# breuner/elbencho

Hardware: AMD Instinct MI355X
Metric: seq-read GiB/s into GPU HBM (higher is better)
Workload: dtype raw-bytes; 1 GPU; seqread; model=storage-benchmark seq-read into HBM, threads_per_gpu=16, block_size=4194304, iodepth=1, bench_dir=/dev/shm/elbencho_amd_bench, gpu_staged=True, mmap_zero_copy=True, dynamic_slice=True, verify_on_gpu=True, verify_salt=7, parallelism=single, device=AMD Radeon Graphics, device_numa_node=0

## Files before the change

elbencho_amd/csrc/engine.cpp:

```cpp

#include "engine.h"

#include <fcntl.h>
#include <linux/fs.h>
#include <pthread.h>
#include <sched.h>
#include <sys/ioctl.h>
#include <sys/mman.h>
#include <sys/stat.h>
#include <sys/types.h>
#include <unistd.h>

#include <algorithm>
#include <random>
#include <cerrno>
#include <cstdio>
#include <cstring>

#include "netbench.h"
#include "uring.h"

namespace eb {

static constexpr uint64_t INTERRUPT_CHECK_INTERVAL = 128;
// ... 884 lines not shown
                if (slotBusy[slot]) gpu->waitSlotEvent(slot);
                if (lat && gpu->timedPairActive(slot))
                    addIoLat(preadUs[slot] + gpu->timedElapsedUSec(slot));

                auto t0 = lat ? Clock::now() : Clock::time_point();
                ssize_t res = pread(fg.fds[fileIdx], hostBufs[slot], ioLen, inFileOff);
                if (res != (ssize_t)ioLen) throwErrno("read", cfg.paths[fileIdx]);
                if (lat) {
                    preadUs[slot] = (uint64_t)std::chrono::duration_cast<
                        std::chrono::microseconds>(Clock::now() - t0).count();
                    gpu->recordTimedStart(slot);
                }

                gpu->copyH2DAsync(slot, ioLen);
                if (lat) gpu->recordTimedEnd(slot);
                if (doVerify) {
                    if ((inFileOff % 8 == 0) && (ioLen % 16 == 0)) {
                        if (eng.verifyMix)
                            gpu->verifyChecksumMixDevAsync(slot, ioLen, inFileOff,
                                                           (uint64_t)cfg.verifySalt,
                                                           cfg.blockSize, eng.verifyMixLen);
                        else
                            gpu->verifyChecksumDevAsync(slot, ioLen, inFileOff,
                                                        (uint64_t)cfg.verifySalt);
                        if (++sinceFetch >= VERIFY_FETCH_INTERVAL) {
                            fetchVerify();
                            sinceFetch = 0;
                        }
                    } else {
                        uint64_t bad =
                            eng.verifyMix
                                ? verifyChecksumMixCPU(hostBufs[slot], ioLen, inFileOff,
                                                       (uint64_t)cfg.verifySalt,
                                                       cfg.blockSize, eng.verifyMixLen)
                                : verifyChecksumCPU(hostBufs[slot], ioLen, inFileOff,
                                                    (uint64_t)cfg.verifySalt);
                        if (bad != UINT64_MAX)
                            throw WorkerError(
                                "Data verification failed. First bad file offset: " +
                                std::to_string(bad));
                    }
                }
                gpu->recordSlotEvent(slot);
                slotBusy[slot] = 1;

                liveOps.bytes.fetch_add(ioLen, std::memory_order_relaxed);
                liveOps.iops.fetch_add(1, std::memory_order_relaxed);
                slot = (slot + 1) % nSlots;
            }
            if (doVerify) fetchVerify();
            if (lat) {
                gpu->syncStream();
                for (int s = 0; s < nSlots; s++)
                    if (gpu->timedPairActive(s))
                        addIoLat(preadUs[s] + gpu->timedElapsedUSec(s));
            }
        }

        gpu->syncStream();
        return;
    }

    const bool lat = cfg.measureLat;
    BlockSpec spec;
    uint64_t opCount = 0;

    while (gen->next(spec)) {
        if ((opCount++ % INTERRUPT_CHECK_INTERVAL) == 0) checkInterrupt();

        uint64_t fileIdx, inFileOff, ioLen;
        if (!mapBlock(spec, fileIdx, inFileOff, ioLen)) continue;

        bool mixRead = rwMixActive &&
                       (isDedicatedReader ||
                        (cfg.rwMixThreads == 0 && rwMixDecideRead()));
        bool blockWrite = isWrite && !mixRead;

        if (rwMixActive && rwBalancerActive()) rwBalanceWait(mixRead, ioLen);

        auto t0 = lat ? Clock::now() : Clock::time_point();

        ssize_t res = blockIO(blockWrite, fg.fds[fileIdx], 0, ioLen, inFileOff,
                              mg.base(fileIdx), &cfg.paths[fileIdx]);
        if (res < 0)
            throwErrno(blockWrite ? "write" : "read", cfg.paths[fileIdx]);
        if ((uint64_t)res != ioLen)
            throw WorkerError(std::string("unexpected short ") + (blockWrite ? "write" : "read") +
                              ". Path: " + cfg.paths[fileIdx] +
                              "; expected: " + std::to_string(ioLen) +
                              "; got: " + std::to_string(res) +
                              (mixRead ? "; Hint: rwmix reads need a pre-written file." : ""));

        if (lat)
            addIoLat((uint64_t)std::chrono::duration_cast<std::chrono::microseconds>(
                Clock::now() - t0).count(), mixRead);

        AtomicLiveOps& ops = mixRead ? liveOpsReadMix : liveOps;
        ops.bytes.fetch_add(ioLen, std::memory_order_relaxed);
        ops.iops.fetch_add(1, std::memory_order_relaxed);
        if (rwMixActive && rwBalancerActive()) rwBalanceAccount(mixRead, ioLen);
    }

    if (isWrite && cfg.fsyncPerFile)
        for (size_t i = 0; i < fg.fds.size(); i++)
            if (fsync(fg.fds[i])) throwErrno("fsync", cfg.paths[i]);
}

void Worker::fileModeBlocksGpuMmap(bool isWrite)
{
    const auto& cfg = eng.cfg;
    const uint64_t fileSize = eng.effFileSize;
    const uint64_t bs = cfg.blockSize;
    const size_t numFiles = cfg.paths.size();
    const uint64_t numBlocksPerFile = (fileSize + bs - 1) / bs;
    const bool doVerify = cfg.verifySalt >= 0;
    const bool lat = cfg.measureLat;

    std::vector<char*> bases(numFiles);
    for (size_t i = 0; i < numFiles; i++)
        bases[i] = eng.getMappedReg(cfg.paths[i], fileSize, isWrite).base;

    const uint64_t mapBPF = (cfg.random || cfg.strided) ? (fileSize / bs) : numBlocksPerFile;
    const uint64_t virtFileLen = mapBPF * bs;

    const bool dynamic = cfg.dynamicSlice && !cfg.random && !cfg.strided &&
                         !cfg.backward && cfg.numThreads == cfg.numDataSetThreads;

    std::unique_ptr<OffsetGen> gen;
    if (dynamic) {
    } else if (cfg.random || cfg.strided) {
        uint64_t numBlocksTotal = mapBPF * numFiles;
        uint64_t rangeLen = bs * (numBlocksTotal / cfg.numDataSetThreads);
        uint64_t rangeOff = (uint64_t)globalRank * rangeLen;
        if (cfg.strided) {
            gen = std::make_unique<OffsetGenStrided>(bs, globalRank, cfg.numDataSetThreads);
            gen->reset(0, bs * numBlocksTotal);
        } else {
            gen = makeOffsetGen(rangeOff, rangeLen);
        }
    } else {
        uint64_t myStart, myLen;
        fairShareSlice(virtFileLen * numFiles, myStart, myLen);
        if (!myLen) return;
        gen = makeOffsetGen(myStart, myLen);
    }

    const int nSlots = (int)hostBufs.size();
    constexpr uint64_t VERIFY_FETCH_INTERVAL = 64;
    uint64_t sinceFetch = 0;
    BlockSpec spec;
    uint64_t opCount = 0;
    int slot = 0;

    auto fetchVerify = [&]() {
        GpuVerifyResult r = gpu->fetchVerifyResult();
        if (r.numMismatches)
            throw WorkerError("Data verification failed (GPU). First bad file offset: " +
                              std::to_string(r.firstBadFileOffset) +
                              "; mismatching 8-byte words: " +
                              std::to_string(r.numMismatches));
    };

    if (doVerify && !isWrite) (void)gpu->fetchVerifyResult();

    const uint64_t totalBlocks = numBlocksPerFile * numFiles;

    auto nextBlock = [&](uint64_t& fileIdx, uint64_t& inFileOff,
                         uint64_t& ioLen) -> bool {
        if (dynamic) {
            for (;;) {
                uint64_t b = eng.dynCursor.fetch_add(1, std::memory_order_relaxed);
                if (b >= totalBlocks) return false;
                fileIdx = b / numBlocksPerFile;
                inFileOff = (b % numBlocksPerFile) * bs;
                if (inFileOff >= fileSize) continue;
                ioLen = std::min(bs, fileSize - inFileOff);
                return true;
            }
        }
        while (gen->next(spec)) {
            if (!virtFileLen) return false;
            fileIdx = spec.offset / virtFileLen;
            if (fileIdx >= numFiles) continue;
            inFileOff = spec.offset - fileIdx * virtFileLen;
            if (inFileOff >= fileSize) continue;
            ioLen = std::min(spec.len, fileSize - inFileOff);
            return true;
        }
        return false;
    };

    uint64_t fileIdx, inFileOff, ioLen;
    while (nextBlock(fileIdx, inFileOff, ioLen)) {
        if ((opCount++ % INTERRUPT_CHECK_INTERVAL) == 0) checkInterrupt();

        rateLimiter.wait(ioLen);

        if (lat && gpu->timedPairActive(slot))
            addIoLat(gpu->timedElapsedUSec(slot));

        if (isWrite) {
            preWriteFill(slot, ioLen, inFileOff);
            if (lat) gpu->recordTimedStart(slot);
            gpu->copyToHostAsync(slot, bases[fileIdx] + inFileOff, ioLen);
            if (lat) gpu->recordTimedEnd(slot);
        } else {
            if (lat) gpu->recordTimedStart(slot);
            gpu->copyFromHostAsync(slot, bases[fileIdx] + inFileOff, ioLen);
            if (lat) gpu->recordTimedEnd(slot);
            if (doVerify && (inFileOff % 8 == 0) && (ioLen % 16 == 0)) {
                if (eng.verifyMix)
                    gpu->verifyChecksumMixDevAsync(slot, ioLen, inFileOff,
                                                   (uint64_t)cfg.verifySalt, cfg.blockSize,
                                                   eng.verifyMixLen);
                else
                    gpu->verifyChecksumDevAsync(slot, ioLen, inFileOff,
                                                (uint64_t)cfg.verifySalt);
                if (++sinceFetch >= VERIFY_FETCH_INTERVAL) {
                    fetchVerify();
                    sinceFetch = 0;
                }
            } else if (doVerify) {
                uint64_t bad =
                    eng.verifyMix
                        ? verifyChecksumMixCPU(bases[fileIdx] + inFileOff, ioLen, inFileOff,
                                               (uint64_t)cfg.verifySalt, cfg.blockSize,
                                               eng.verifyMixLen)
                        : verifyChecksumCPU(bases[fileIdx] + inFileOff, ioLen, inFileOff,
                                            (uint64_t)cfg.verifySalt);
                if (bad != UINT64_MAX)
                    throw WorkerError("Data verification failed. First bad file offset: " +
                                      std::to_string(bad));
            }
        }

        liveOps.bytes.fetch_add(ioLen, std::memory_order_relaxed);
        liveOps.iops.fetch_add(1, std::memory_order_relaxed);
        slot = (slot + 1) % nSlots;

        if ((opCount & 127) == 0) gpu->syncStream();
    }

    gpu->syncStream();
    if (lat)
        for (int s = 0; s < nSlots; s++)
            if (gpu->timedPairActive(s)) addIoLat(gpu->timedElapsedUSec(s));
    if (doVerify && !isWrite) fetchVerify();
}

void Worker::fileModeBlocksUring(bool isWrite)
{
    const auto& cfg = eng.cfg;
    const uint64_t fileSize = eng.effFileSize;
    const uint64_t bs = cfg.blockSize;
    const size_t numFiles = cfg.paths.size();
    const uint64_t numBlocksPerFile = (fileSize + bs - 1) / bs;
    const int depth = cfg.ioDepth;
    const bool lat = cfg.measureLat;

    const bool rwMixActive = isWrite && (cfg.rwMixPct > 0 || isDedicatedReader);

    FdGuard fg;
    int rwFlags = isWrite ? ((cfg.verifyDirect || rwMixActive) ? O_RDWR : O_WRONLY) : O_RDONLY;
    int openFlags = rwFlags | (cfg.directIO ? O_DIRECT : 0);
    if (isWrite && cfg.pathType == PathType::FILE) openFlags |= O_CREAT;
    for (const auto& p : cfg.paths) {
        int fd = open(p.c_str(), openFlags, 0644);
        if (fd < 0) throwErrno("open", p);
        fg.fds.push_back(fd);
        if (isWrite && cfg.pathType == PathType::FILE) {
            if (cfg.truncate && ftruncate(fd, 0)) throwErrno("truncate", p);
            if (cfg.truncToSize != UINT64_MAX && ftruncate(fd, fileSize))
                throwErrno("truncate-to-size", p);
            if (cfg.preallocFile && fallocate(fd, 0, 0, fileSize)) throwErrno("fallocate", p);
        }
        applyFadvise(fd, cfg.fadviseFlags, p);
    }

    const uint64_t mapBPF = (cfg.random || cfg.strided) ? (fileSize / bs) : numBlocksPerFile;
    const uint64_t virtFileLen = mapBPF * bs;

    auto mapBlock = [&](const BlockSpec& s, uint64_t& fileIdx, uint64_t& inFileOff,
                        uint64_t& ioLen) -> bool {
        if (!virtFileLen) return false;
        fileIdx = s.offset / virtFileLen;
        if (fileIdx >= numFiles) return false;
        inFileOff = s.offset - fileIdx * virtFileLen;
        if (inFileOff >= fileSize) return false;
        ioLen = std::min(s.len, fileSize - inFileOff);
        return true;
    };

    std::unique_ptr<OffsetGen> gen;
    if (cfg.random || cfg.strided) {
        uint64_t numBlocksTotal = mapBPF * numFiles;
        uint64_t rangeLen = bs * (numBlocksTotal / cfg.numDataSetThreads);
        uint64_t rangeOff = (uint64_t)globalRank * rangeLen;
        if (cfg.strided) {
            gen = std::make_unique<OffsetGenStrided>(bs, globalRank, cfg.numDataSetThreads);
            gen->reset(0, bs * numBlocksTotal);
        } else {
            gen = makeOffsetGen(rangeOff, rangeLen);
        }
    } else {
        uint64_t myStart, myLen;
        fairShareSlice(virtFileLen * numFiles, myStart, myLen);
        if (!myLen) return;
        gen = makeOffsetGen(myStart, myLen);
    }

    IoUring ring;
    ring.init(depth);

    if (!getenv("EB_URING_NOFIXED")) {
        std::vector<struct iovec> iovs(depth);
        for (int s = 0; s < depth; s++)
            iovs[s] = {hostBufs[s], (size_t)bs};
        ring.registerBuffers(iovs.data(), depth);
        ring.registerFiles(fg.fds.data(), (unsigned)fg.fds.size());
    }

    const int gpuBatch = gpu ? gpuBatchSlots(bs) : 1;
    const bool batchedRead = gpu && !isWrite && cfg.verifySalt < 0 &&
                             gpuBatch >= 2 && depth >= 4 &&
                             getenv("EB_GPU_URING_BATCH");
    if (getenv("EB_DEBUG_PATH"))
        fprintf(stderr, "[eb] uring path: gpu=%d batchedRead=%d batch=%d depth=%d\n",
                gpu ? 1 : 0, (int)batchedRead, gpuBatch, depth);
    if (batchedRead) {
        const int halfSize = std::min(depth / 2, 64);
        struct Op {
            uint64_t off = 0, len = 0;
            Clock::time_point start;
            int fileIdx = 0;
        };
        std::vector<Op> ops(2 * halfSize);
        std::vector<IoUring::Completion> bcomps(depth);
        int submitted[2] = {0, 0}, done[2] = {0, 0};
        bool exhausted2 = false;
        BlockSpec bspec;

        auto fillHalf = [&](int h) -> int {
            int base = h * halfSize;
            int n = 0;
            while (n < halfSize && !exhausted2) {
                uint64_t fileIdx = 0, inFileOff = 0, ioLen = 0;
                for (;;) {
                    if (!gen->next(bspec)) { exhausted2 = true; break; }
                    if (mapBlock(bspec, fileIdx, inFileOff, ioLen)) break;
                }
                if (exhausted2) break;
                rateLimiter.wait(ioLen);
                int slot = base + n;
                ops[slot] = {inFileOff, ioLen,
                             lat ? Clock::now() : Clock::time_point(), (int)fileIdx};
                if (eng.opsLog.isEnabled())
                    eng.opsLog.log(globalRank, "uring_read", cfg.paths[fileIdx],
                                   inFileOff, ioLen, true, false);
                int rfd = ring.hasFixedFiles() ? (int)fileIdx : fg.fds[fileIdx];
                while (!ring.prep(false, rfd, hostBufs[slot], ioLen, inFileOff,
                                  (uint64_t)slot,
                                  ring.hasFixedBuffers() ? slot : -1,
                                  ring.hasFixedFiles())) {
                    ring.submitAndWait(0);
                    checkInterrupt();
                }
                n++;
            }
            submitted[h] = n;
            done[h] = 0;
            return n;
        };

        int inFlightB = fillHalf(0) + fillHalf(1);
        uint64_t opCountB = 0;
        while (inFlightB > 0) {
            checkInterrupt();
            ring.submitAndWait(1, 250);
            unsigned n = ring.reap(bcomps.data(), depth);
            for (unsigned i = 0; i < n; i++) {
                int slot = (int)bcomps[i].userData;
                const Op& op = ops[slot];
                if (eng.opsLog.isEnabled())
                    eng.opsLog.log(globalRank, "uring_read", cfg.paths[op.fileIdx],
                                   op.off, op.len, false, bcomps[i].res < 0);
                if (bcomps[i].res < 0)
                    throw WorkerError(std::string("async read failed. Path: ") +
                                      cfg.paths[op.fileIdx] + "; SysErr: " +
                                      strerror(-bcomps[i].res));
                if ((uint64_t)bcomps[i].res != op.len)
                    throw WorkerError("unexpected short async read. Path: " +
                                      cfg.paths[op.fileIdx]);
                if (lat)
                    addIoLat((uint64_t)std::chrono::duration_cast<
                        std::chrono::microseconds>(Clock::now() - op.start).count());
                liveOps.bytes.fetch_add(op.len, std::memory_order_relaxed);
                liveOps.iops.fetch_add(1, std::memory_order_relaxed);
                done[slot / halfSize]++;
                inFlightB--;
                if ((opCountB++ % INTERRUPT_CHECK_INTERVAL) == 0) checkInterrupt();
// ... 1752 lines not shown
```

elbencho_amd/csrc/gpu.h:

```cpp

#pragma once

#include <cstdint>
#include <string>
#include <vector>

#include "crc.h"

namespace eb {

struct GpuVerifyResult {
    uint64_t numMismatches;
    uint64_t firstBadFileOffset;
};

void gpuHostRegister(void* ptr, uint64_t len);
bool gpuHostRegisterTry(void* ptr, uint64_t len);
void gpuHostUnregister(void* ptr);

class GpuCtx;

int gpuDeviceCount();

double gpuVerifyBenchGBs(uint64_t len, int iters, bool lds, int dev);

double gpuMixBenchGBs(uint64_t len, int iters, int dev, uint64_t blockSize, uint64_t mixLen,
                      bool fill, bool plainFill);

uint64_t gpuCrcTileBytes();
uint64_t gpuCrcWaveBytes();

std::string gpuProbeError();

std::string gpuDeviceName(int deviceId);

int gpuNumaNode(int deviceId);

class GpuCtx {
public:
    GpuCtx(int deviceId, int numSlots, uint64_t bufSize, bool pinnedHostBufs);
    ~GpuCtx();
    GpuCtx(const GpuCtx&) = delete;
    GpuCtx& operator=(const GpuCtx&) = delete;

    int deviceId() const { return devId; }
    char* hostBuf(int slot) const;
    uint64_t bufSize() const { return slotSize; }
    int numSlots() const { return slots; }
    uint64_t slotStride() const;

    void snapshotSlots(std::vector<char>& dst);

    void bindThread();

    void copyFromHostAsync(int slot, const void* src, uint64_t len);
    void copyToHostAsync(int slot, void* dst, uint64_t len);
    void copyH2DAsync(int slot, uint64_t len);
    void copyH2DRangeAsync(int firstSlot, int count);
    void copyD2HAsync(int slot, uint64_t len);
    void syncStream();

    void recordSlotEvent(int slot);
    void waitSlotEvent(int slot);

    void recordTimedStart(int slot);
    void recordTimedEnd(int slot);
    bool timedPairActive(int slot) const;
    uint64_t timedElapsedUSec(int slot);
    void dropTimedPairs();

    void verifyChecksumDevAsync(int slot, uint64_t len, uint64_t fileOff, uint64_t salt,
                                bool ldsVariant = false);
    GpuVerifyResult fetchVerifyResult();


    void fillRandDev(int slot, uint64_t len, uint64_t seed, bool fastAlgo = false);

    void fillChecksumDev(int slot, uint64_t len, uint64_t fileOff, uint64_t salt);

    GpuVerifyResult verifyChecksumDev(int slot, uint64_t len, uint64_t fileOff, uint64_t salt,
                                      bool ldsVariant = false);

    void fillChecksumMixDev(int slot, uint64_t len, uint64_t fileOff, uint64_t salt,
                            uint64_t blockSize, uint64_t mixLen);
    void verifyChecksumMixDevAsync(int slot, uint64_t len, uint64_t fileOff, uint64_t salt,
                                   uint64_t blockSize, uint64_t mixLen);
    GpuVerifyResult verifyChecksumMixDev(int slot, uint64_t len, uint64_t fileOff,
                                         uint64_t salt, uint64_t blockSize, uint64_t mixLen);

    void blockVarRefillDev(int slot, uint64_t len, uint64_t refillLen, uint64_t seed,
                           bool fastAlgo = false);


    void crcDevAsync(int slot, uint64_t len, CrcAlgo algo, uint64_t partialBase);

    uint32_t crcFetch(CrcAlgo algo, uint64_t totalLen, uint64_t tileCount);

    uint32_t crcDev(int slot, uint64_t len, CrcAlgo algo);

private:
    struct Impl;
    Impl* impl;
    int devId;
    uint64_t slotSize;
    int slots;
};

}
```

elbencho_amd/csrc/gpu_kernels.hip:

```cpp

#include <hip/hip_runtime.h>

#include <cstdio>
#include <map>
#include <mutex>
#include <stdexcept>
#include <string>
#include <vector>

#include "crc.h"
#include "gpu.h"

namespace eb {

#define HIP_CHECK(cmd)                                                                 \
    do {                                                                               \
        hipError_t e = (cmd);                                                          \
        if (e != hipSuccess)                                                           \
            throw std::runtime_error(std::string("HIP error: ") + hipGetErrorString(e) \
                                     + " at " __FILE__ ":" + std::to_string(__LINE__)); \
    } while (0)


__device__ __forceinline__ uint64_t d_splitmix64(uint64_t& state)
// ... 388 lines not shown
        ((uint4*)tab)[i] = ((const uint4*)tables)[i];
    __syncthreads();

    constexpr uint64_t TILE_VEC2 = CRC_TILE_BYTES / 16;
    const uint64_t nTiles = (nVec2 + TILE_VEC2 - 1) / TILE_VEC2;
    const int wave = threadIdx.x >> 6;
    const int lane = threadIdx.x & 63;

    for (uint64_t tile = blockIdx.x; tile < nTiles; tile += gridDim.x) {
        const uint64_t first = tile * TILE_VEC2;
        const uint64_t have = (nVec2 - first < TILE_VEC2) ? nVec2 - first : TILE_VEC2;
        const uint64_t pad = TILE_VEC2 - have;

        ulonglong2 v[CRC_STEPS_PER_WAVE];
#pragma unroll
        for (int j = 0; j < CRC_STEPS_PER_WAVE; j++) {
            uint64_t pos = (uint64_t)(wave * CRC_STEPS_PER_WAVE + j) * 64 + lane;
            v[j] = make_ulonglong2(0, 0);
            if (pos >= pad) v[j] = buf[first + pos - pad];
        }

        uint32_t acc = 0;
#pragma unroll
        for (int j = 0; j < CRC_STEPS_PER_WAVE; j++) {
            uint32_t r = 0;
#pragma unroll
            for (int k = 0; k < 8; k++) {
                r ^= tab[(CRC_TAB_ELEM + k) * 256 + ((v[j].x >> (8 * k)) & 0xFF)];
                r ^= tab[(CRC_TAB_ELEM + 8 + k) * 256 + ((v[j].y >> (8 * k)) & 0xFF)];
            }
            acc = d_crcLut4(tab + CRC_TAB_ROW * 256, acc) ^ r;
        }

#pragma unroll
        for (int i = 0; i < 6; i++) {
            uint32_t other = __shfl_down(acc, 1 << i, 64);
            acc = d_crcLut4(tab + (CRC_TAB_LANE + 4 * i) * 256, acc) ^ other;
        }

        if (lane == 0) wavePart[wave] = acc;
        __syncthreads();
        if (threadIdx.x == 0) {
            uint32_t t = 0;
#pragma unroll
            for (int w = 0; w < CRC_WAVES_PER_TILE; w++)
                t = d_crcLut4(tab + CRC_TAB_WAVE * 256, t) ^ wavePart[w];
            partial[tile] = t;
        }
        __syncthreads();
    }
}


double gpuVerifyBenchGBs(uint64_t len, int iters, bool lds, int dev);

bool gpuHostRegisterTry(void* ptr, uint64_t len)
{
    return hipHostRegister(ptr, len, hipHostRegisterDefault) == hipSuccess;
}

void gpuHostRegister(void* ptr, uint64_t len)
{
    HIP_CHECK(hipHostRegister(ptr, len, hipHostRegisterDefault));
}

void gpuHostUnregister(void* ptr) { (void)hipHostUnregister(ptr); }

int gpuDeviceCount()
{
    int n = 0;
    hipError_t e = hipGetDeviceCount(&n);
    if (e != hipSuccess) return 0;
    return n;
}

std::string gpuProbeError()
{
    int n = 0;
    hipError_t e = hipGetDeviceCount(&n);
    if (e != hipSuccess) return hipGetErrorString(e);
    return "ok: " + std::to_string(n) + " device(s)";
}

std::string gpuDeviceName(int deviceId)
{
    hipDeviceProp_t prop;
    if (hipGetDeviceProperties(&prop, deviceId) != hipSuccess) return "";
    return prop.name;
}

int gpuNumaNode(int deviceId)
{
    char busId[32] = {0};
    if (hipDeviceGetPCIBusId(busId, sizeof(busId), deviceId) != hipSuccess)
        return -1;
    for (char* c = busId; *c; ++c) *c = (char)tolower(*c);
    std::string path = std::string("/sys/bus/pci/devices/") + busId + "/numa_node";
    FILE* f = fopen(path.c_str(), "r");
    if (!f) return -1;
    int node = -1;
    if (fscanf(f, "%d", &node) != 1) node = -1;
    fclose(f);
    return node;
}

static dim3 gridForBytes(uint64_t workItems)
{
    uint64_t blocks = (workItems + 255) / 256;
    if (blocks > 4096) blocks = 4096;
    if (blocks == 0) blocks = 1;
    return dim3((uint32_t)blocks);
}

static hipStream_t sharedStream(int devId, int& poolSizeOut)
{
    static std::mutex mtx;
    static std::map<int, std::vector<hipStream_t>> pools;
    static std::map<int, int> next;
    static const int poolSize = [] {
        const char* v = getenv("EB_GPU_SHARED_STREAMS");
        int n = v ? atoi(v) : 8;
        return (n >= 1 && n <= 64) ? n : 0;
    }();

    poolSizeOut = poolSize;
    if (!poolSize) return nullptr;

    std::lock_guard<std::mutex> lk(mtx);
    auto& pool = pools[devId];
    if (pool.empty()) {
        pool.resize(poolSize);
        for (int i = 0; i < poolSize; i++)
            HIP_CHECK(hipStreamCreateWithFlags(&pool[i], hipStreamNonBlocking));
    }
    return pool[next[devId]++ % poolSize];
}

struct GpuCtx::Impl {
    hipStream_t stream = nullptr;
    bool ownStream = true;
    char* devBase = nullptr;
    char* hostBase = nullptr;
    uint64_t slotStride = 0;
    std::vector<char*> devBufs;
    std::vector<char*> hostBufs;
    std::vector<hipEvent_t> slotEvents;
    std::vector<hipEvent_t> timedStart, timedEnd;
    std::vector<char> timedActive;
    bool hostPinned = false;
    unsigned long long* verifyOutDev = nullptr;
    unsigned long long* verifyOutHost = nullptr;
    uint64_t fillCallCounter = 0;
    bool verifyDirty = false;

    uint32_t* crcTabDev[2] = {nullptr, nullptr};
    CrcShift crcTileShift[2];
    uint32_t* crcPartDev = nullptr;
    uint32_t* crcPartHost = nullptr;
    uint64_t crcPartCap = 0;
    struct CrcCall { uint64_t base, len; };
    std::vector<CrcCall> crcPending;
};

GpuCtx::GpuCtx(int deviceId, int numSlots, uint64_t bufSize, bool pinnedHostBufs)
    : impl(new Impl), devId(deviceId), slotSize(bufSize), slots(numSlots)
{
    HIP_CHECK(hipSetDevice(deviceId));
    int poolSize = 0;
    hipStream_t shared = sharedStream(deviceId, poolSize);
    if (shared) {
        impl->stream = shared;
        impl->ownStream = false;
    } else {
        HIP_CHECK(hipStreamCreateWithFlags(&impl->stream, hipStreamNonBlocking));
    }

    impl->hostPinned = pinnedHostBufs;
    impl->devBufs.resize(numSlots, nullptr);
    impl->hostBufs.resize(numSlots, nullptr);

    impl->slotStride = (bufSize + 4095) & ~4095ULL;
    HIP_CHECK(hipMalloc(&impl->devBase, impl->slotStride * numSlots));
    if (pinnedHostBufs) {
        static const unsigned hostFlags = [] {
            const char* v = getenv("EB_GPU_HOSTALLOC");
            return (v && v[0] == 'n') ? hipHostMallocNonCoherent : hipHostMallocDefault;
        }();
        HIP_CHECK(hipHostMalloc(&impl->hostBase, impl->slotStride * numSlots, hostFlags));
    } else {
        if (posix_memalign((void**)&impl->hostBase, 4096, impl->slotStride * numSlots))
            throw std::runtime_error("host buffer alloc failed");
    }
    for (int i = 0; i < numSlots; i++) {
        impl->devBufs[i] = impl->devBase + (uint64_t)i * impl->slotStride;
        impl->hostBufs[i] = impl->hostBase + (uint64_t)i * impl->slotStride;
    }

    impl->slotEvents.resize(numSlots, nullptr);
    static const bool evBlock = [] {
        const char* v = getenv("EB_GPU_EVBLOCK");
        return v && v[0] == '1';
    }();
    unsigned evFlags = hipEventDisableTiming | (evBlock ? hipEventBlockingSync : 0);
    for (int i = 0; i < numSlots; i++)
        HIP_CHECK(hipEventCreateWithFlags(&impl->slotEvents[i], evFlags));

    HIP_CHECK(hipMalloc(&impl->verifyOutDev, 2 * sizeof(unsigned long long)));
    HIP_CHECK(hipHostMalloc(&impl->verifyOutHost, 2 * sizeof(unsigned long long),
                            hipHostMallocDefault));

    impl->verifyOutHost[0] = 0;
    impl->verifyOutHost[1] = ~0ULL;
    HIP_CHECK(hipMemcpy(impl->verifyOutDev, impl->verifyOutHost,
                        2 * sizeof(unsigned long long), hipMemcpyHostToDevice));
}

GpuCtx::~GpuCtx()
{
    (void)hipSetDevice(devId);
    if (impl->devBase) (void)hipFree(impl->devBase);
    if (impl->hostBase) {
        if (impl->hostPinned)
            (void)hipHostFree(impl->hostBase);
        else
            free(impl->hostBase);
    }
    for (auto e : impl->slotEvents)
        if (e) (void)hipEventDestroy(e);
    for (auto e : impl->timedStart)
        if (e) (void)hipEventDestroy(e);
    for (auto e : impl->timedEnd)
        if (e) (void)hipEventDestroy(e);
    if (impl->verifyOutDev) (void)hipFree(impl->verifyOutDev);
    if (impl->verifyOutHost) (void)hipHostFree(impl->verifyOutHost);
    for (auto p : impl->crcTabDev)
        if (p) (void)hipFree(p);
    if (impl->crcPartDev) (void)hipFree(impl->crcPartDev);
    if (impl->crcPartHost) (void)hipHostFree(impl->crcPartHost);
    if (impl->stream && impl->ownStream) (void)hipStreamDestroy(impl->stream);
    delete impl;
}

char* GpuCtx::hostBuf(int slot) const { return impl->hostBufs[slot]; }

void GpuCtx::bindThread() { HIP_CHECK(hipSetDevice(devId)); }

uint64_t GpuCtx::slotStride() const { return impl->slotStride; }

void GpuCtx::snapshotSlots(std::vector<char>& dst)
{
    dst.resize(impl->slotStride * (uint64_t)slots);
    if (dst.empty()) return;
    HIP_CHECK(hipMemcpyAsync(dst.data(), impl->devBase, dst.size(), hipMemcpyDeviceToHost,
                             impl->stream));
    HIP_CHECK(hipStreamSynchronize(impl->stream));
}

void GpuCtx::copyFromHostAsync(int slot, const void* src, uint64_t len)
{
    HIP_CHECK(hipMemcpyAsync(impl->devBufs[slot], src, len, hipMemcpyHostToDevice,
                             impl->stream));
}

void GpuCtx::copyToHostAsync(int slot, void* dst, uint64_t len)
{
    HIP_CHECK(hipMemcpyAsync(dst, impl->devBufs[slot], len, hipMemcpyDeviceToHost,
                             impl->stream));
}

void GpuCtx::copyH2DAsync(int slot, uint64_t len)
{
    HIP_CHECK(hipMemcpyAsync(impl->devBufs[slot], impl->hostBufs[slot], len,
                             hipMemcpyHostToDevice, impl->stream));
}

void GpuCtx::copyH2DRangeAsync(int firstSlot, int count)
{
    HIP_CHECK(hipMemcpyAsync(impl->devBufs[firstSlot], impl->hostBufs[firstSlot],
                             impl->slotStride * count, hipMemcpyHostToDevice,
                             impl->stream));
}

void GpuCtx::copyD2HAsync(int slot, uint64_t len)
{
    HIP_CHECK(hipMemcpyAsync(impl->hostBufs[slot], impl->devBufs[slot], len,
                             hipMemcpyDeviceToHost, impl->stream));
}

void GpuCtx::syncStream() { HIP_CHECK(hipStreamSynchronize(impl->stream)); }

void GpuCtx::recordSlotEvent(int slot)
{
    HIP_CHECK(hipEventRecord(impl->slotEvents[slot], impl->stream));
}

void GpuCtx::waitSlotEvent(int slot)
{
    HIP_CHECK(hipEventSynchronize(impl->slotEvents[slot]));
}


void GpuCtx::recordTimedStart(int slot)
{
    if (impl->timedStart.empty()) {
        impl->timedStart.resize(slots, nullptr);
        impl->timedEnd.resize(slots, nullptr);
        impl->timedActive.assign(slots, 0);
        for (int i = 0; i < slots; i++) {
            HIP_CHECK(hipEventCreateWithFlags(&impl->timedStart[i], hipEventDefault));
            HIP_CHECK(hipEventCreateWithFlags(&impl->timedEnd[i], hipEventDefault));
        }
    }
    HIP_CHECK(hipEventRecord(impl->timedStart[slot], impl->stream));
}

void GpuCtx::recordTimedEnd(int slot)
{
    HIP_CHECK(hipEventRecord(impl->timedEnd[slot], impl->stream));
    impl->timedActive[slot] = 1;
}

bool GpuCtx::timedPairActive(int slot) const
{
    return !impl->timedActive.empty() && impl->timedActive[slot];
}

uint64_t GpuCtx::timedElapsedUSec(int slot)
{
    HIP_CHECK(hipEventSynchronize(impl->timedEnd[slot]));
    float ms = 0;
    HIP_CHECK(hipEventElapsedTime(&ms, impl->timedStart[slot], impl->timedEnd[slot]));
    impl->timedActive[slot] = 0;
    return (uint64_t)(ms * 1000.0f);
}

void GpuCtx::dropTimedPairs()
{
    for (auto& a : impl->timedActive) a = 0;
}

static void requireAligned(const char* what, uint64_t len, uint64_t lenAlign,
                           uint64_t fileOff = 0)
{
    if (len % lenAlign)
        throw std::invalid_argument(std::string(what) + ": len " + std::to_string(len) +
                                    " is not a multiple of " + std::to_string(lenAlign));
    if (fileOff % 8)
        throw std::invalid_argument(std::string(what) + ": fileOff " +
                                    std::to_string(fileOff) + " is not a multiple of 8");
}

void GpuCtx::verifyChecksumDevAsync(int slot, uint64_t len, uint64_t fileOff, uint64_t salt,
                                    bool ldsVariant)
{
    requireAligned("verifyChecksumDev", len, 8, fileOff);
    uint64_t n64 = len / 8;
    if (!n64) return;
    dim3 grid = gridForBytes(n64 / 2);
    if (ldsVariant)
        hipLaunchKernelGGL(ebVerifyChecksumLdsKernel, grid, dim3(256), 0, impl->stream,
                           (const ulonglong2*)impl->devBufs[slot], n64, fileOff, salt,
                           impl->verifyOutDev);
    else
        hipLaunchKernelGGL(ebVerifyChecksumKernel, grid, dim3(256), 0, impl->stream,
                           (const ulonglong2*)impl->devBufs[slot], n64, fileOff, salt,
                           impl->verifyOutDev);
    HIP_CHECK(hipGetLastError());
    impl->verifyDirty = true;
}

GpuVerifyResult GpuCtx::fetchVerifyResult()
{
    if (!impl->verifyDirty) return GpuVerifyResult{0, ~0ULL};
    HIP_CHECK(hipMemcpyAsync(impl->verifyOutHost, impl->verifyOutDev,
                             2 * sizeof(unsigned long long), hipMemcpyDeviceToHost,
                             impl->stream));
    HIP_CHECK(hipStreamSynchronize(impl->stream));
    GpuVerifyResult r{impl->verifyOutHost[0], impl->verifyOutHost[1]};
    impl->verifyOutHost[0] = 0;
    impl->verifyOutHost[1] = ~0ULL;
    HIP_CHECK(hipMemcpyAsync(impl->verifyOutDev, impl->verifyOutHost,
                             2 * sizeof(unsigned long long), hipMemcpyHostToDevice,
                             impl->stream));
    HIP_CHECK(hipStreamSynchronize(impl->stream));
    impl->verifyDirty = false;
    return r;
}

void GpuCtx::fillRandDev(int slot, uint64_t len, uint64_t seed, bool fastAlgo)
{
    requireAligned("fillRandDev", len, 16);
    uint64_t nVec2 = len / 16;
    uint64_t seq = ++impl->fillCallCounter;
    if (nVec2) {
        if (fastAlgo) {
            dim3 grid = gridForBytes(nVec2);
            hipLaunchKernelGGL(ebFillFastKernel, grid, dim3(256), 0, impl->stream,
                               (ulonglong2*)impl->devBufs[slot], nVec2,
                               seed + seq * 0x9E3779B9ULL);
        } else {
            dim3 grid = gridForBytes(nVec2 / (FILL_U64S_PER_STEP / 2));
            hipLaunchKernelGGL(ebFillRandKernel, grid, dim3(256), 0, impl->stream,
                               (ulonglong2*)impl->devBufs[slot], nVec2,
                               seed + seq * 0x9E3779B9ULL);
        }
        HIP_CHECK(hipGetLastError());
    }
}

void GpuCtx::fillChecksumDev(int slot, uint64_t len, uint64_t fileOff, uint64_t salt)
{
    requireAligned("fillChecksumDev", len, 8, fileOff);
    uint64_t n64 = len / 8;
    if (!n64) return;
    dim3 grid = gridForBytes(n64);
    hipLaunchKernelGGL(ebFillChecksumKernel, grid, dim3(256), 0, impl->stream,
                       (uint64_t*)impl->devBufs[slot], n64, fileOff, salt);
    HIP_CHECK(hipGetLastError());
}

GpuVerifyResult GpuCtx::verifyChecksumDev(int slot, uint64_t len, uint64_t fileOff, uint64_t salt,
                                          bool ldsVariant)
{
    verifyChecksumDevAsync(slot, len, fileOff, salt, ldsVariant);
    return fetchVerifyResult();
}

static void requireMixGeometry(const char* what, uint64_t len, uint64_t blockSize,
                               uint64_t mixLen)
{
    if (!blockSize || blockSize % 8)
        throw std::invalid_argument(std::string(what) + ": block size " +
                                    std::to_string(blockSize) +
                                    " is not a positive multiple of 8");
    if (mixLen % 8)
        throw std::invalid_argument(std::string(what) + ": mix length " +
                                    std::to_string(mixLen) + " is not a multiple of 8");
    if (mixLen > blockSize)
        throw std::invalid_argument(std::string(what) + ": mix length " +
                                    std::to_string(mixLen) + " exceeds the block size " +
                                    std::to_string(blockSize));
    if (len > blockSize)
        throw std::invalid_argument(std::string(what) + ": len " + std::to_string(len) +
                                    " exceeds the block size " + std::to_string(blockSize));
}

void GpuCtx::fillChecksumMixDev(int slot, uint64_t len, uint64_t fileOff, uint64_t salt,
                                uint64_t blockSize, uint64_t mixLen)
{
    requireAligned("fillChecksumMixDev", len, 8, fileOff);
    requireMixGeometry("fillChecksumMixDev", len, blockSize, mixLen);
    if (len > impl->slotStride)
        throw std::invalid_argument("fillChecksumMixDev: len " + std::to_string(len) +
                                    " exceeds the slot size");
    uint64_t n64 = len / 8;
    if (!n64) return;
    dim3 grid = gridForBytes(n64);
    hipLaunchKernelGGL(ebFillChecksumMixKernel, grid, dim3(256), 0, impl->stream,
                       (uint64_t*)impl->devBufs[slot], n64, fileOff, salt,
                       fileOff % blockSize, blockSize, mixLen);
    HIP_CHECK(hipGetLastError());
}

void GpuCtx::verifyChecksumMixDevAsync(int slot, uint64_t len, uint64_t fileOff,
                                       uint64_t salt, uint64_t blockSize, uint64_t mixLen)
{
    requireAligned("verifyChecksumMixDev", len, 8, fileOff);
    requireMixGeometry("verifyChecksumMixDev", len, blockSize, mixLen);
    if (len > impl->slotStride)
        throw std::invalid_argument("verifyChecksumMixDev: len " + std::to_string(len) +
                                    " exceeds the slot size");
    uint64_t n64 = len / 8;
    if (!n64) return;
    dim3 grid = gridForBytes(n64 / 2);
    hipLaunchKernelGGL(ebVerifyChecksumMixKernel, grid, dim3(256), 0, impl->stream,
                       (const ulonglong2*)impl->devBufs[slot], n64, fileOff, salt,
                       fileOff % blockSize, blockSize, mixLen, impl->verifyOutDev);
    HIP_CHECK(hipGetLastError());
    impl->verifyDirty = true;
}

GpuVerifyResult GpuCtx::verifyChecksumMixDev(int slot, uint64_t len, uint64_t fileOff,
                                             uint64_t salt, uint64_t blockSize,
                                             uint64_t mixLen)
{
    verifyChecksumMixDevAsync(slot, len, fileOff, salt, blockSize, mixLen);
    return fetchVerifyResult();
}

void GpuCtx::blockVarRefillDev(int slot, uint64_t len, uint64_t refillLen, uint64_t seed,
                               bool fastAlgo)
{
    requireAligned("blockVarRefillDev", len, 16);
    uint64_t nVec2 = len / 16;
    if (!nVec2) return;
    uint64_t refillVec2 = refillLen / 16;
    uint64_t seq = ++impl->fillCallCounter;
    uint64_t sm = seed + seq;
    uint64_t z = (sm += 0x9E3779B97F4A7C15ULL);
    z = (z ^ (z >> 30)) * 0xBF58476D1CE4E5B9ULL;
    z = (z ^ (z >> 27)) * 0x94D049BB133111EBULL;
    uint64_t fillConst = z ^ (z >> 31);

    if (fastAlgo) {
        dim3 grid = gridForBytes(nVec2);
        hipLaunchKernelGGL(ebBlockVarFastKernel, grid, dim3(256), 0, impl->stream,
                           (ulonglong2*)impl->devBufs[slot], nVec2, refillVec2,
                           seed + seq * 0x9E3779B9ULL, fillConst);
    } else {
        dim3 grid = gridForBytes(nVec2 / (FILL_U64S_PER_STEP / 2));
        hipLaunchKernelGGL(ebBlockVarKernel, grid, dim3(256), 0, impl->stream,
                           (ulonglong2*)impl->devBufs[slot], nVec2, refillVec2,
                           seed + seq * 0x9E3779B9ULL, fillConst);
    }
    HIP_CHECK(hipGetLastError());
}


uint64_t gpuCrcTileBytes() { return CRC_TILE_BYTES; }
uint64_t gpuCrcWaveBytes() { return CRC_WAVE_BYTES; }

void GpuCtx::crcDevAsync(int slot, uint64_t len, CrcAlgo algo, uint64_t partialBase)
{
    requireAligned("crcDevAsync", len, 16);
    if (len > impl->slotStride)
        throw std::invalid_argument("crcDevAsync: len " + std::to_string(len) +
                                    " exceeds the slot size");
    if (!len) return;
    const int a = (int)algo;
    const uint64_t tiles = (len + CRC_TILE_BYTES - 1) / CRC_TILE_BYTES;

    if (!impl->crcTabDev[a]) {
        std::vector<uint32_t> tab = crcBuildTileTables(algo, CRC_STEPS_PER_WAVE);
        HIP_CHECK(hipMalloc(&impl->crcTabDev[a], tab.size() * sizeof(uint32_t)));
        HIP_CHECK(hipMemcpy(impl->crcTabDev[a], tab.data(), tab.size() * sizeof(uint32_t),
                            hipMemcpyHostToDevice));
        impl->crcTileShift[a] = CrcShift(algo, CRC_TILE_BYTES);
    }

    if (partialBase + tiles > impl->crcPartCap) {
        uint64_t cap = std::max<uint64_t>(4096, impl->crcPartCap * 2);
        while (cap < partialBase + tiles) cap *= 2;
        uint32_t* dev = nullptr;
        uint32_t* host = nullptr;
        HIP_CHECK(hipMalloc(&dev, cap * sizeof(uint32_t)));
        HIP_CHECK(hipHostMalloc(&host, cap * sizeof(uint32_t), hipHostMallocDefault));
        if (impl->crcPartDev) {
            HIP_CHECK(hipStreamSynchronize(impl->stream));
            HIP_CHECK(hipMemcpy(dev, impl->crcPartDev, impl->crcPartCap * sizeof(uint32_t),
                                hipMemcpyDeviceToDevice));
            (void)hipFree(impl->crcPartDev);
            (void)hipHostFree(impl->crcPartHost);
        }
        impl->crcPartDev = dev;
        impl->crcPartHost = host;
        impl->crcPartCap = cap;
    }

    dim3 grid = gridForBytes(tiles * 256);
    hipLaunchKernelGGL(ebCrcTilesKernel, grid, dim3(256), 0, impl->stream,
                       (const ulonglong2*)impl->devBufs[slot], len / 16,
                       (const uint32_t*)impl->crcTabDev[a], impl->crcPartDev + partialBase);
    HIP_CHECK(hipGetLastError());
    impl->crcPending.push_back({partialBase, len});
}

uint32_t GpuCtx::crcFetch(CrcAlgo algo, uint64_t totalLen, uint64_t tileCount)
{
    std::vector<Impl::CrcCall> calls;
    calls.swap(impl->crcPending);
    uint64_t tiles = 0, bytes = 0;
    for (const auto& c : calls) {
        if (c.base != tiles)
            throw std::invalid_argument("crcFetch: partials are not contiguous in call order");
        tiles += (c.len + CRC_TILE_BYTES - 1) / CRC_TILE_BYTES;
        bytes += c.len;
    }
    if (tiles != tileCount || bytes != totalLen)
        throw std::invalid_argument("crcFetch: " + std::to_string(tileCount) + " tiles / " +
                                    std::to_string(totalLen) + " bytes asked, " +
                                    std::to_string(tiles) + " / " + std::to_string(bytes) +
                                    " enqueued");
    if (!tileCount) return crcFinishRaw(algo, 0, 0);

    HIP_CHECK(hipMemcpyAsync(impl->crcPartHost, impl->crcPartDev, tileCount * sizeof(uint32_t),
                             hipMemcpyDeviceToHost, impl->stream));
    HIP_CHECK(hipStreamSynchronize(impl->stream));

    const CrcShift& tileShift = impl->crcTileShift[(int)algo];
    const uint32_t* part = impl->crcPartHost;
    uint32_t raw = 0;
    for (const auto& c : calls) {
        const uint64_t full = c.len / CRC_TILE_BYTES;
        for (uint64_t i = 0; i < full; i++) raw = tileShift.apply(raw) ^ *part++;
        if (c.len % CRC_TILE_BYTES) raw = crcCombine(algo, raw, *part++, c.len % CRC_TILE_BYTES);
    }
    return crcFinishRaw(algo, raw, totalLen);
}

uint32_t GpuCtx::crcDev(int slot, uint64_t len, CrcAlgo algo)
{
    impl->crcPending.clear();
    crcDevAsync(slot, len, algo, 0);
    return crcFetch(algo, len, (len + CRC_TILE_BYTES - 1) / CRC_TILE_BYTES);
}

double gpuVerifyBenchGBs(uint64_t len, int iters, bool lds, int dev)
{
    HIP_CHECK(hipSetDevice(dev));
    const uint64_t n64 = len / 8;
    ulonglong2* buf = nullptr;
    unsigned long long* out = nullptr;
    HIP_CHECK(hipMalloc(&buf, len));
    HIP_CHECK(hipMalloc(&out, 2 * sizeof(unsigned long long)));
    HIP_CHECK(hipMemset(out, 0, 2 * sizeof(unsigned long long)));

    hipStream_t s;
    HIP_CHECK(hipStreamCreateWithFlags(&s, hipStreamNonBlocking));
    dim3 grid = gridForBytes(n64 / 2);

    hipLaunchKernelGGL(ebFillChecksumKernel, gridForBytes(len / 8), dim3(256), 0, s,
                       (uint64_t*)buf, len / 8, 0, 7);

    auto launch = [&] {
        if (lds)
            hipLaunchKernelGGL(ebVerifyChecksumLdsKernel, grid, dim3(256), 0, s,
                               buf, n64, 0, 7, out);
        else
            hipLaunchKernelGGL(ebVerifyChecksumKernel, grid, dim3(256), 0, s,
                               buf, n64, 0, 7, out);
    };

// ... 81 lines not shown
```

Measured before the change: 52.17 GiB/s.

## Replace periodic stream syncs with per-slot events and async verify snapshots

On the read path, the full stream synchronize every 128 ops and the blocking verify fetch (two memcpys, two syncs, resetting the counter) are replaced. The new code records an event per slot and waits only before reusing that slot. It also takes double-buffered asynchronous snapshots of the verify counters, so verification no longer drains the pipeline. The verify accumulator is no longer reset between windows, so mismatch counts become cumulative. Error detection is deferred by one window.

```diff
diff --git a/elbencho_amd/csrc/engine.cpp b/elbencho_amd/csrc/engine.cpp
--- a/elbencho_amd/csrc/engine.cpp
+++ b/elbencho_amd/csrc/engine.cpp
@@ -1060,13 +1060,21 @@
     uint64_t opCount = 0;
     int slot = 0;
 
-    auto fetchVerify = [&]() {
-        GpuVerifyResult r = gpu->fetchVerifyResult();
+    std::vector<char> slotPending(nSlots, 0);
+    int pendingSnap = -1;
+
+    auto checkVerify = [](const GpuVerifyResult& r) {
         if (r.numMismatches)
             throw WorkerError("Data verification failed (GPU). First bad file offset: " +
                               std::to_string(r.firstBadFileOffset) +
                               "; mismatching 8-byte words: " +
                               std::to_string(r.numMismatches));
+    };
+    auto collectSnapshot = [&]() {
+        if (pendingSnap < 0) return;
+        int id = pendingSnap;
+        pendingSnap = -1;
+        checkVerify(gpu->waitVerifySnapshot(id));
     };
 
     if (doVerify && !isWrite) (void)gpu->fetchVerifyResult();
@@ -1106,6 +1114,10 @@
 
         if (lat && gpu->timedPairActive(slot))
             addIoLat(gpu->timedElapsedUSec(slot));
+        if (slotPending[slot]) {
+            gpu->waitSlotEvent(slot);
+            slotPending[slot] = 0;
+        }
 
         if (isWrite) {
             preWriteFill(slot, ioLen, inFileOff);
@@ -1125,10 +1137,12 @@
                     gpu->verifyChecksumDevAsync(slot, ioLen, inFileOff,
                                                 (uint64_t)cfg.verifySalt);
                 if (++sinceFetch >= VERIFY_FETCH_INTERVAL) {
-                    fetchVerify();
+                    collectSnapshot();
+                    pendingSnap = gpu->snapshotVerifyAsync();
                     sinceFetch = 0;
                 }
             } else if (doVerify) {
+                collectSnapshot();
                 uint64_t bad =
                     eng.verifyMix
                         ? verifyChecksumMixCPU(bases[fileIdx] + inFileOff, ioLen, inFileOff,
@@ -1144,16 +1158,27 @@
 
         liveOps.bytes.fetch_add(ioLen, std::memory_order_relaxed);
         liveOps.iops.fetch_add(1, std::memory_order_relaxed);
+        if (!lat && !isWrite) {
+            gpu->recordSlotEvent(slot);
+            slotPending[slot] = 1;
+        }
         slot = (slot + 1) % nSlots;
 
-        if ((opCount & 127) == 0) gpu->syncStream();
-    }
-
-    gpu->syncStream();
-    if (lat)
-        for (int s = 0; s < nSlots; s++)
-            if (gpu->timedPairActive(s)) addIoLat(gpu->timedElapsedUSec(s));
-    if (doVerify && !isWrite) fetchVerify();
+        if (isWrite && (opCount & 127) == 0) gpu->syncStream();
+    }
+
+    if (isWrite) gpu->syncStream();
+
+    GpuVerifyResult lastWindow{0, UINT64_MAX}, rest{0, UINT64_MAX};
+    const int restSnap = (doVerify && !isWrite && sinceFetch) ? gpu->snapshotVerifyAsync() : -1;
+    if (pendingSnap >= 0) lastWindow = gpu->waitVerifySnapshot(pendingSnap);
+    if (restSnap >= 0) rest = gpu->waitVerifySnapshot(restSnap);
+    for (int s = 0; s < nSlots; s++) {
+        if (lat && gpu->timedPairActive(s)) addIoLat(gpu->timedElapsedUSec(s));
+        if (slotPending[s]) gpu->waitSlotEvent(s);
+    }
+    checkVerify(lastWindow);
+    checkVerify(rest);
 }
 
 void Worker::fileModeBlocksUring(bool isWrite)
diff --git a/elbencho_amd/csrc/gpu.h b/elbencho_amd/csrc/gpu.h
--- a/elbencho_amd/csrc/gpu.h
+++ b/elbencho_amd/csrc/gpu.h
@@ -73,6 +73,10 @@
                                 bool ldsVariant = false);
     GpuVerifyResult fetchVerifyResult();
 
+    static constexpr int VERIFY_SNAPSHOTS = 2;
+    int snapshotVerifyAsync();
+    GpuVerifyResult waitVerifySnapshot(int id);
+
 
     void fillRandDev(int slot, uint64_t len, uint64_t seed, bool fastAlgo = false);
 
diff --git a/elbencho_amd/csrc/gpu_kernels.hip b/elbencho_amd/csrc/gpu_kernels.hip
--- a/elbencho_amd/csrc/gpu_kernels.hip
+++ b/elbencho_amd/csrc/gpu_kernels.hip
@@ -564,6 +564,11 @@
     unsigned long long* verifyOutHost = nullptr;
     uint64_t fillCallCounter = 0;
     bool verifyDirty = false;
+    unsigned long long* verifySnapHost = nullptr;
+    hipEvent_t verifySnapEvents[GpuCtx::VERIFY_SNAPSHOTS] = {};
+    uint64_t verifySnapSeq[GpuCtx::VERIFY_SNAPSHOTS] = {};
+    uint64_t verifyLaunchSeq = 0;
+    int verifySnapNext = 0;
 
     uint32_t* crcTabDev[2] = {nullptr, nullptr};
     CrcShift crcTileShift[2];
@@ -620,6 +625,11 @@
     HIP_CHECK(hipMalloc(&impl->verifyOutDev, 2 * sizeof(unsigned long long)));
     HIP_CHECK(hipHostMalloc(&impl->verifyOutHost, 2 * sizeof(unsigned long long),
                             hipHostMallocDefault));
+    HIP_CHECK(hipHostMalloc(&impl->verifySnapHost,
+                            VERIFY_SNAPSHOTS * 2 * sizeof(unsigned long long),
+                            hipHostMallocDefault));
+    for (int i = 0; i < VERIFY_SNAPSHOTS; i++)
+        HIP_CHECK(hipEventCreateWithFlags(&impl->verifySnapEvents[i], evFlags));
 
     impl->verifyOutHost[0] = 0;
     impl->verifyOutHost[1] = ~0ULL;
@@ -645,6 +655,9 @@
         if (e) (void)hipEventDestroy(e);
     if (impl->verifyOutDev) (void)hipFree(impl->verifyOutDev);
     if (impl->verifyOutHost) (void)hipHostFree(impl->verifyOutHost);
+    if (impl->verifySnapHost) (void)hipHostFree(impl->verifySnapHost);
+    for (auto e : impl->verifySnapEvents)
+        if (e) (void)hipEventDestroy(e);
     for (auto p : impl->crcTabDev)
         if (p) (void)hipFree(p);
     if (impl->crcPartDev) (void)hipFree(impl->crcPartDev);
@@ -779,6 +792,7 @@
                            impl->verifyOutDev);
     HIP_CHECK(hipGetLastError());
     impl->verifyDirty = true;
+    impl->verifyLaunchSeq++;
 }
 
 GpuVerifyResult GpuCtx::fetchVerifyResult()
@@ -799,6 +813,30 @@
     return r;
 }
 
+int GpuCtx::snapshotVerifyAsync()
+{
+    const int id = impl->verifySnapNext;
+    impl->verifySnapNext = (id + 1) % VERIFY_SNAPSHOTS;
+    HIP_CHECK(hipMemcpyAsync(impl->verifySnapHost + 2 * id, impl->verifyOutDev,
+                             2 * sizeof(unsigned long long), hipMemcpyDeviceToHost,
+                             impl->stream));
+    HIP_CHECK(hipEventRecord(impl->verifySnapEvents[id], impl->stream));
+    impl->verifySnapSeq[id] = impl->verifyLaunchSeq;
+    return id;
+}
+
+GpuVerifyResult GpuCtx::waitVerifySnapshot(int id)
+{
+    if (id < 0 || id >= VERIFY_SNAPSHOTS)
+        throw std::invalid_argument("waitVerifySnapshot: bad snapshot id " +
+                                    std::to_string(id));
+    HIP_CHECK(hipEventSynchronize(impl->verifySnapEvents[id]));
+    GpuVerifyResult r{impl->verifySnapHost[2 * id], impl->verifySnapHost[2 * id + 1]};
+    if (!r.numMismatches && impl->verifySnapSeq[id] == impl->verifyLaunchSeq)
+        impl->verifyDirty = false;
+    return r;
+}
+
 void GpuCtx::fillRandDev(int slot, uint64_t len, uint64_t seed, bool fastAlgo)
 {
     requireAligned("fillRandDev", len, 16);
@@ -890,6 +928,7 @@
                        fileOff % blockSize, blockSize, mixLen, impl->verifyOutDev);
     HIP_CHECK(hipGetLastError());
     impl->verifyDirty = true;
+    impl->verifyLaunchSeq++;
 }
 
 GpuVerifyResult GpuCtx::verifyChecksumMixDev(int slot, uint64_t len, uint64_t fileOff,
```

Result: no change. 52.22 GiB/s (median of 2 runs) (+0.1%).
